# thu-nics/Rad-NeRF

Hardware: AMD Instinct MI355X
Metric: million samples/s fwd+bwd, 8192 rays, model_zoo_size=2; rgb L∞ vs ref (higher is better)
Workload: dtype f16/f32

## Files before the change

rad-nerf_amd/csrc/field_fwd_merged.hip:

```cpp
#include "rn_field.h"
#include "rn_merge.h"
#pragma clang fp contract(off)

static uint64_t g_level_pairing = 0;

namespace {

#define FM_KMAX 8
#define FM_LDS_K 4
static_assert(FM_KMAX == MB_KMAX, "k_field_fwd_merged reads the plan's descriptors");

template <int CACHE, bool ENC_M, bool GW>
__global__ void __launch_bounds__(1024)
k_field_fwd_merged(FieldArgs a, MergeArgs m) {
    extern __shared__ __attribute__((aligned(16))) rn_half sWm[];
    __shared__ LvTab sT;
    __shared__ int32_t sCh[2][2 + 2 * FM_KMAX];
    const int K = m.n_models, B = m.n_rays;
    if (!GW) {
        for (int k = 0; k < K; ++k)
            rn_block_copy16(sWm + (size_t)k * FIELD_FWD_FRAGS * RN_FRAG_HALFS,
                            a.frags + (size_t)k * FIELD_FRAGS * RN_FRAG_HALFS,
                            FIELD_FWD_FRAGS * RN_FRAG_BYTES);
    }
    lv_stage(sT, a.gm);
    const int waves = blockDim.x / RN_WAVE;
    const int wid = __builtin_amdgcn_readfirstlane(threadIdx.x / RN_WAVE);
    const int lane = rn_lane(), c = lane & 31, h = lane >> 5;
    int ticket = 0, n_chunks = 0;
    if (threadIdx.x == 0) { n_chunks = m.queue[1]; ticket = atomicAdd(m.queue + 2, 1); }

    auto mlp_tile = [&](const int32_t* ch, int u) {
        const int k = u % K, t = u / K;
        const int n_k = ch[2 + FM_KMAX + k];
        if (t * 32 >= n_k) return;
        rn_lds_order();
        const int i = t * 32 + c;
        const bool valid = i < n_k;
        const int64_t s = ch[2 + k] + (valid ? i : 0);
        FwdState st;
        float ux, uy, uz;
        constexpr int TC = ENC_M ? CACHE_READ_NT : CACHE;
        const rn_half* W = GW ? a.frags + (size_t)k * FIELD_FRAGS * RN_FRAG_HALFS
                              : sWm + (size_t)k * FIELD_FWD_FRAGS * RN_FRAG_HALFS;
        tile_forward_s<1, TC>(a, sT, W, s, valid, TC != CACHE_NONE ? cache_slot(a, s) : nullptr,
                              st, ux, uy, uz);
        if (valid && h == 0) {
            a.sigma[s] = expf(st.g0);
            a.rgb[3 * s + 0] = sigmoidf(st.out[0]);
            a.rgb[3 * s + 1] = sigmoidf(st.out[1]);
            a.rgb[3 * s + 2] = sigmoidf(st.out[2]);
        }
    };
    auto mlp_tiles = [&](const int32_t* ch) {
        int max_t = 0;
        for (int k = 0; k < K; ++k) max_t = max(max_t, (ch[2 + FM_KMAX + k] + 31) >> 5);
        return max_t * K;
    };

    bool prev_live = false;
    for (int it = 0;; ++it) {
        int32_t* cur = sCh[it & 1];
        const int32_t* prev = sCh[(it & 1) ^ 1];
        __syncthreads();
        if (threadIdx.x == 0) {
            const int ch = ticket;
            ticket = atomicAdd(m.queue + 2, 1);
            int4 d[CH_DESC / 4];
            if (ch < n_chunks) {
#pragma unroll
                for (int q = 0; q < CH_DESC / 4; ++q)
                    d[q] = reinterpret_cast<const int4*>(m.desc + (size_t)ch * CH_DESC)[q];
            }
            const int32_t* di = reinterpret_cast<const int32_t*>(d);
            cur[0] = ch < n_chunks ? di[CH_R0] : B;
            cur[1] = ch < n_chunks ? di[CH_R1] : B;
            for (int k = 0; k < K; ++k) {
                cur[2 + k] = di[ch_first(k)];
                cur[2 + FM_KMAX + k] = ch < n_chunks ? di[ch_count(k)] : 0;
            }
        }
        __syncthreads();
        const bool live = cur[0] < B;
        if (!ENC_M) {
            if (!live) break;
            const int nt = mlp_tiles(cur);
            for (int u = wid; u < nt; u += waves) mlp_tile(cur, u);
            continue;
        }
        if (!live && !prev_live) break;
        int p_base = 0, n_p = 0;
        if (live) { p_base = m.mstart[cur[0]]; n_p = m.mstart[cur[1]] - p_base; }
        const int nA = (n_p + 31) >> 5;
        const int nB = prev_live ? mlp_tiles(prev) : 0;
        for (int u = wid; u < nA + nB; u += waves) {
            if (u >= nA) { mlp_tile(prev, u - nA); continue; }
            const int q = u * 32 + c;
            const bool valid = q < n_p;
            const int64_t s = m.perm[p_base + (valid ? q : 0)];
            float x, y, z, dx, dy, dz;
            load_sample<1>(a, s, x, y, z, dx, dy, dz);
            const float ux = unit_coord(x, a.xyz_min[0], a.extent[0]);
            const float uy = unit_coord(y, a.xyz_min[1], a.extent[1]);
            const float uz = unit_coord(z, a.xyz_min[2], a.extent[2]);
            half8 e0, e1;
            encode_lane(a, sT, rn_rsrc(a.grid, a.grid_bytes), h, ux, uy, uz, valid, e0, e1);
            if (valid) { half8* fc = cache_slot(a, s); fc[0] = e0; fc[1] = e1; }
        }
        prev_live = live;
    }
}


__global__ void __launch_bounds__(256)
k_enc_prep(FieldArgs a, MergeArgs m, float4* __restrict__ prep) {
    const int P = m.mstart[m.n_rays];
    for (int p = blockIdx.x * blockDim.x + threadIdx.x; p < P; p += gridDim.x * blockDim.x) {
        const int s = m.perm[p];
        float x, y, z, dx, dy, dz;
        load_sample<1>(a, s, x, y, z, dx, dy, dz);
        prep[p] = make_float4(unit_coord(x, a.xyz_min[0], a.extent[0]),
                              unit_coord(y, a.xyz_min[1], a.extent[1]),
                              unit_coord(z, a.xyz_min[2], a.extent[2]), __int_as_float(s));
    }
}

__global__ void __launch_bounds__(256)
k_field_encode_levels(FieldArgs a, MergeArgs m, const float4* __restrict__ prep,
                      int32_t* __restrict__ xq, uint64_t pairing) {
    __shared__ LvTab sT;
    lv_stage(sT, a.gm);
    __syncthreads();
    const int g = blockIdx.x & 7;
    if (xq && threadIdx.x == 0) {
        uint32_t xcc;
        asm volatile("s_getreg_b32 %0, hwreg(HW_REG_XCC_ID, 0, 4)" : "=s"(xcc));
        atomicAdd(xq + 8 * g + (int)(xcc & 7u), 1);
        atomicMin(reinterpret_cast<unsigned long long*>(xq + 64) + g,
                  (unsigned long long)__builtin_amdgcn_s_memrealtime());
    }
    const int la = (int)((pairing >> (8 * g)) & 15u), lb = (int)((pairing >> (8 * g + 4)) & 15u);
    const int P = m.mstart[m.n_rays];
    const int nt = (P + 31) >> 5;
    const int nb = (int)(gridDim.x >> 3), j = (int)(blockIdx.x >> 3);
    const int t0 = (int)((int64_t)nt * j / nb), t1 = (int)((int64_t)nt * (j + 1) / nb);
    const int wid = __builtin_amdgcn_readfirstlane(threadIdx.x >> 6), waves = blockDim.x >> 6;
    const int lane = rn_lane(), c = lane & 31, h = lane >> 5;
    const __amdgpu_buffer_rsrc_t rs = rn_rsrc(a.grid, a.grid_bytes);
    const LvConst LA = lv_const_uniform(sT, a.gm, la), LB = lv_const_uniform(sT, a.gm, lb);
#pragma unroll 1
    for (int ph = 0; ph < 2; ++ph) {
        const LvConst& LC = ph ? LB : LA;
        uint32_t* const out = const_cast<uint32_t*>(a.planes) + (size_t)(ph ? lb : la) * a.plane_stride;
        for (int t = t0 + 2 * wid; t < t1; t += 2 * waves) {
            const bool v0 = t * 32 + c < P;
            const bool v1 = t + 1 < t1 && (t + 1) * 32 + c < P;
            const bool valid = h ? v1 : v0;
            const int p = (t + h) * 32 + c;
            const float4 q = prep[valid ? p : 0];
            const uint32_t v = encode_tiles(a, rs, h, LC, q.x, q.y, q.z, v0, v1);
            if (valid) __builtin_nontemporal_store(v, out + __float_as_int(q.w));
        }
    }
    if (xq) {
        __syncthreads();
        if (threadIdx.x == 0)
            atomicMax(reinterpret_cast<unsigned long long*>(xq + 80) + g,
                      (unsigned long long)__builtin_amdgcn_s_memrealtime());
    }
}

__global__ void __launch_bounds__(1024)
k_field_mlp_planes(FieldArgs a, int K) {
    extern __shared__ __attribute__((aligned(16))) rn_half sWm[];
    __shared__ LvTab sT;
    __shared__ int32_t sSeg[2][FM_KMAX];
    lv_stage(sT, a.gm);
    if (threadIdx.x < K) {
        sSeg[0][threadIdx.x] = a.seg_base[threadIdx.x];
        sSeg[1][threadIdx.x] = a.seg_count[threadIdx.x];
    }
    int first[FM_KMAX + 1];
    first[0] = 0;
    for (int k = 0; k < K; ++k)
        first[k + 1] = first[k] + ((__builtin_amdgcn_readfirstlane(a.seg_count[k]) + 31) >> 5);
    const int T = first[K];
    const int u0 = (int)((int64_t)T * blockIdx.x / gridDim.x);
    const int u1 = (int)((int64_t)T * (blockIdx.x + 1) / gridDim.x);
    if (u0 >= u1) return;
    int k_lo = 0, k_hi = 0;
    for (int k = 0; k < K; ++k) {
        if (first[k + 1] <= u0) k_lo = k + 1;
        if (first[k] < u1) k_hi = k;
    }
    const int wid = __builtin_amdgcn_readfirstlane(threadIdx.x >> 6), waves = blockDim.x >> 6;
    const int lane = rn_lane(), c = lane & 31, h = lane >> 5;
    for (int kb = k_lo; kb <= k_hi; kb += FM_LDS_K) {
        const int ke = min(k_hi, kb + FM_LDS_K - 1);
        __syncthreads();
        for (int k = kb; k <= ke; ++k)
            rn_block_copy16(sWm + (size_t)(k - kb) * FIELD_FWD_FRAGS * RN_FRAG_HALFS,
                            a.frags + (size_t)k * FIELD_FRAGS * RN_FRAG_HALFS,
                            FIELD_FWD_FRAGS * RN_FRAG_BYTES);
        __syncthreads();
        const int ua = max(u0, first[kb]), ub = min(u1, first[ke + 1]);
        for (int u = ua + wid; u < ub; u += waves) {
            int k = kb;
            while (k < ke && u >= first[k + 1]) ++k;
            const int t = u - first[k];
            const int n_k = sSeg[1][k];
            const int i = t * 32 + c;
            const bool valid = i < n_k;
            const int64_t s = sSeg[0][k] + (valid ? i : 0);
            FwdState st;
            float ux, uy, uz;
            rn_lds_order();
            tile_forward_s<1, CACHE_PLANES>(a, sT, sWm + (size_t)(k - kb) * FIELD_FWD_FRAGS * RN_FRAG_HALFS,
                                            s, valid, a.feat ? cache_slot(a, s) : nullptr, st,
                                            ux, uy, uz);
            if (valid && h == 0) {
                a.sigma[s] = expf(st.g0);
                a.rgb[3 * s + 0] = sigmoidf(st.out[0]);
                a.rgb[3 * s + 1] = sigmoidf(st.out[1]);
                a.rgb[3 * s + 2] = sigmoidf(st.out[2]);
            }
        }
    }
}

}

extern "C" {

int rn_set_level_pairing(uint64_t pairing) {
    if (pairing != 0) {
        uint32_t seen = 0;
        for (int i = 0; i < 16; ++i) seen |= 1u << ((pairing >> (4 * i)) & 15u);
        RN_CHECK_ARG(seen == 0xffffu, "pairing: every level exactly once");
    }
    g_level_pairing = pairing;
    return 0;
}

int rn_field_fwd_merged(const float* ts, const int32_t* ray_of, const float* rays_o,
                        const float* rays_d, const int32_t* seg_base, const int32_t* seg_count,
                        const int32_t* chunk_desc, int32_t* queue,
                        int64_t n_rays, int32_t n_models, const void* grid_f16,
                        const uint32_t* level_offset, const uint32_t* level_hsize,
                        const uint32_t* level_res, const float* level_scale,
                        const float* xyz_min, const float* extent, const void* frags,
                        float* sigma, float* rgb, void* feat_cache, const int32_t* mstart,
                        const int32_t* perm, int32_t blocks, int32_t threads, void* stream) {
    RN_CHECK_ARG(n_rays >= 1 && n_models >= 1 && n_models <= FM_KMAX && blocks >= 1,
                 "bad sizes (n_models <= 8)");
    RN_CHECK_ARG(threads >= 64 && threads <= 1024 && threads % 64 == 0, "threads: 64..1024, waves");
    RN_CHECK_ARG(ts && ray_of && rays_o && rays_d && seg_base && seg_count &&
                 chunk_desc && queue && grid_f16 && level_offset && level_hsize && level_res &&
                 level_scale && xyz_min && extent && frags && sigma && rgb, "null pointer");
    RN_CHECK_ARG(!(mstart || perm) || (mstart && perm && feat_cache),
                 "merged-order encoding needs mstart, perm and the encoding cache");
    FieldArgs a{};
    field_args_grid(a, grid_f16, level_offset, level_hsize, level_res, level_scale, xyz_min, extent,
                    frags);
    field_args_compact(a, ts, ray_of, rays_o, rays_d, seg_base, seg_count);
    a.sigma = sigma; a.rgb = rgb; a.feat = (rn_half*)feat_cache;
    MergeArgs m{};
    m.desc = chunk_desc; m.queue = queue;
    m.mstart = mstart; m.perm = perm;
    m.n_rays = (int)n_rays; m.n_models = n_models;
    const bool gw = n_models > FM_LDS_K;
    const size_t lds = gw ? 0 : (size_t)n_models * FIELD_FWD_FRAGS * RN_FRAG_BYTES;
    hipStream_t st = (hipStream_t)stream;
    RN_CHECK_HIP(hipMemsetAsync(queue + 2, 0, sizeof(int32_t), st), "ticket reset");
#define RN_FM_LAUNCH(C, E)                                                                     \
    do {                                                                                       \
        if (gw) k_field_fwd_merged<C, E, true><<<blocks, threads, 0, st>>>(a, m);              \
        else k_field_fwd_merged<C, E, false><<<blocks, threads, lds, st>>>(a, m);              \
    } while (0)
    if (mstart) RN_FM_LAUNCH(CACHE_WRITE, true);
    else if (feat_cache) RN_FM_LAUNCH(CACHE_WRITE, false);
    else RN_FM_LAUNCH(CACHE_NONE, false);
#undef RN_FM_LAUNCH
    RN_CHECK_LAUNCH();
    return 0;
}

int rn_field_fwd_levels(const float* ts, const int32_t* ray_of, const float* rays_o,
                        const float* rays_d, const int32_t* seg_base, const int32_t* seg_count,
                        int64_t n_rays, int32_t n_models, const void* grid_f16,
                        const uint32_t* level_offset, const uint32_t* level_hsize,
                        const uint32_t* level_res, const float* level_scale,
                        const float* xyz_min, const float* extent, const void* frags,
                        float* sigma, float* rgb, void* feat_cache, const int32_t* mstart,
                        const int32_t* perm, uint32_t* planes, int64_t plane_stride, void* prep,
                        int32_t prep_ready, int32_t enc_blocks, int32_t mlp_blocks, int32_t* xq,
                        void* stream) {
    RN_CHECK_ARG(n_rays >= 1 && n_models >= 1 && n_models <= FM_KMAX && plane_stride >= 1,
                 "bad sizes (n_models <= 8)");
    RN_CHECK_ARG(enc_blocks >= 8 && enc_blocks % 8 == 0 && mlp_blocks >= 1,
                 "bad launch (enc_blocks: a multiple of 8)");
    RN_CHECK_ARG(ts && ray_of && rays_o && rays_d && seg_base && seg_count && grid_f16 &&
                 level_offset && level_hsize && level_res && level_scale && xyz_min && extent &&
                 frags && sigma && rgb && mstart && perm && planes && prep, "null pointer");
    FieldArgs a{};
    field_args_grid(a, grid_f16, level_offset, level_hsize, level_res, level_scale, xyz_min, extent,
                    frags);
    field_args_compact(a, ts, ray_of, rays_o, rays_d, seg_base, seg_count);
    a.sigma = sigma; a.rgb = rgb; a.feat = (rn_half*)feat_cache;
    a.planes = planes; a.plane_stride = plane_stride;
    MergeArgs m{};
    m.mstart = mstart; m.perm = perm; m.n_rays = (int)n_rays; m.n_models = n_models;
    hipStream_t st = (hipStream_t)stream;
    if (xq) {
        RN_CHECK_HIP(hipMemsetAsync(xq, 0, 64 * sizeof(int32_t), st), "probe reset");
        RN_CHECK_HIP(hipMemsetAsync(xq + 64, 0xff, 16 * sizeof(int32_t), st), "probe reset");
        RN_CHECK_HIP(hipMemsetAsync(xq + 80, 0, 16 * sizeof(int32_t), st), "probe reset");
    }
    if (!prep_ready) k_enc_prep<<<1024, 256, 0, st>>>(a, m, (float4*)prep);
    uint64_t pairing = g_level_pairing;
    if (pairing == 0)
        for (int g = 0; g < 8; ++g) pairing |= (uint64_t)(g | ((RN_L - 1 - g) << 4)) << (8 * g);
    k_field_encode_levels<<<enc_blocks, 256, 0, st>>>(a, m, (const float4*)prep, xq, pairing);
    k_field_mlp_planes<<<mlp_blocks, 1024,
                         (size_t)min(n_models, FM_LDS_K) * FIELD_FWD_FRAGS * RN_FRAG_BYTES, st>>>(
        a, n_models);
    RN_CHECK_LAUNCH();
    return 0;
}

}
```

rad-nerf_amd/csrc/rn_field.h:

```cpp
#pragma once
#include "rn_mlp.h"
#pragma clang fp contract(off)

#define RN_L 16
#define FIELD_FWD_FRAGS 24
#define FIELD_FRAGS 46
#define FIELD_PARAMS 9472
#define FIELD_DW_TILES 12
#ifndef FWD_MIN_WAVES
#define FWD_MIN_WAVES 2
#endif

struct GridMeta {
    uint32_t offset[RN_L];
    uint32_t hsize[RN_L];
    uint32_t res[RN_L];
    float scale[RN_L];
    uint32_t dense_mask;
    uint32_t pow2_mask;
};

struct FieldArgs {
    const float* xyzs; const float* dirs;
    const float* ts; const int32_t* ray_of; const float* rays_o; const float* rays_d;
    const int32_t* seg_base; const int32_t* seg_count;
    int64_t n_fixed;
    const rn_half* grid;
    float* grid_grad;
    const rn_half* frags;
    float* dw;
    float* sigma; float* rgb;
    const float* dsigma; const float* drgb;
    rn_half* feat;
    const uint32_t* planes;
    int64_t plane_stride;
    float xyz_min[3]; float extent[3];
    uint32_t grid_bytes;
    int dbg;
    GridMeta gm;
};

namespace {


__device__ __forceinline__ void sample_range(const FieldArgs& a, int MODE, int k, int64_t& base,
                                             int64_t& n) {
    if (MODE == 0) { base = 0; n = a.n_fixed; }
    else { base = a.seg_base[k]; n = a.seg_count[k]; }
}

template <int MODE>
__device__ __forceinline__ void load_sample(const FieldArgs& a, int64_t s, float& x, float& y,
                                            float& z, float& dx, float& dy, float& dz) {
    if (MODE == 0) {
        x = a.xyzs[3 * s]; y = a.xyzs[3 * s + 1]; z = a.xyzs[3 * s + 2];
        dx = a.dirs[3 * s]; dy = a.dirs[3 * s + 1]; dz = a.dirs[3 * s + 2];
    } else {
        const int r = (rn_dbg(a.dbg) & 8192) ? 0 : a.ray_of[s];
        const float t = a.ts[s];
        dx = a.rays_d[3 * r]; dy = a.rays_d[3 * r + 1]; dz = a.rays_d[3 * r + 2];
        x = fmaf(t, dx, a.rays_o[3 * r]);
        y = fmaf(t, dy, a.rays_o[3 * r + 1]);
        z = fmaf(t, dz, a.rays_o[3 * r + 2]);
    }
}

__device__ __forceinline__ float unit_coord(float v, float mn, float ext) {
    return fminf(fmaxf((v - mn) / ext, 0.0f), 1.0f);
}

__device__ __forceinline__ int lane_level(int q, int h) { return 2 * h + (q & 1) + 4 * (q >> 1); }

struct LvTab {
    uint32_t off[RN_L];
    uint32_t hs[RN_L];
    uint32_t res[RN_L];
    uint32_t res2[RN_L];
    float sc[RN_L];
};

__device__ __forceinline__ void lv_stage(LvTab& t, const GridMeta& gm) {
    const int i = threadIdx.x;
    if (i < RN_L) {
        t.off[i] = gm.offset[i]; t.hs[i] = gm.hsize[i]; t.res[i] = gm.res[i]; t.sc[i] = gm.scale[i];
        t.res2[i] = gm.res[i] * gm.res[i];
    }
}

struct LvConst {
    uint32_t off, hs, res, res2;
    float sc;
    bool dense;
};

__device__ __forceinline__ LvConst lv_const(const LvTab& T, const GridMeta& gm, int l) {
    LvConst c;
    c.off = T.off[l]; c.hs = T.hs[l]; c.res = T.res[l]; c.res2 = T.res2[l]; c.sc = T.sc[l];
    c.dense = (gm.dense_mask >> l) & 1u;
    return c;
}

__device__ __forceinline__ uint32_t grid_index(const LvConst& c, uint32_t x, uint32_t y, uint32_t z) {
    const uint32_t di = x + __umul24(y, c.res) + __umul24(z, c.res2);
    const uint32_t hi = x ^ (y * 2654435761u) ^ (z * 805459861u);
    const uint32_t dm = di >= c.hs ? di - c.hs : di;
    return c.dense ? dm : (hi & (c.hs - 1u));
}

struct LevelPos { uint32_t gx, gy, gz; float fx, fy, fz; };

__device__ __forceinline__ LevelPos level_pos(float sc, float ux, float uy, float uz) {
    LevelPos p;
    float px = fmaf(sc, ux, 0.5f), py = fmaf(sc, uy, 0.5f), pz = fmaf(sc, uz, 0.5f);
    auto cvt_flr = [](float v) {
        int r;
        asm("v_cvt_flr_i32_f32 %0, %1" : "=v"(r) : "v"(v));
        return (uint32_t)r;
    };
    p.gx = cvt_flr(px); p.gy = cvt_flr(py); p.gz = cvt_flr(pz);
    p.fx = __builtin_amdgcn_fractf(px); p.fy = __builtin_amdgcn_fractf(py); p.fz = __builtin_amdgcn_fractf(pz);
    return p;
}

__device__ __forceinline__ float corner_weight(const LevelPos& p, int c) {
    float w = 1.0f;
    w *= (c & 1) ? p.fx : 1.0f - p.fx;
    w *= (c & 2) ? p.fy : 1.0f - p.fy;
    w *= (c & 4) ? p.fz : 1.0f - p.fz;
    return w;
}

__device__ __forceinline__ uint32_t corner_index(const LvConst& c, const LevelPos& p, int corner) {
    return grid_index(c, p.gx + (corner & 1), p.gy + ((corner >> 1) & 1), p.gz + ((corner >> 2) & 1));
}

__device__ __forceinline__ __amdgpu_buffer_rsrc_t rn_rsrc(const void* p, uint32_t bytes) {
    return __builtin_amdgcn_make_buffer_rsrc(const_cast<void*>(p), (short)0, (int)bytes,
                                             0x00020000);
}

#define RN_OOB 0x80000000u

__device__ __forceinline__ void encode_lane(const FieldArgs& a, const LvTab& T,
                                            __amdgpu_buffer_rsrc_t rs, int h, float ux, float uy,
                                            float uz, bool valid, half8& e0, half8& e1) {
    float f[16];
    const bool load = valid && !(rn_dbg(a.dbg) & 128);
#pragma unroll
    for (int lb = 0; lb < RN_L; lb += 4) {
        uint32_t GX[4], ROW[4][4];
        float FX[4], FY[4], FZ[4];
#pragma unroll
        for (int up = 0; up < 4; up += 2) {
            const LvConst lm = lv_const(T, a.gm, lb + up + h);
            const LevelPos p = level_pos(lm.sc, ux, uy, uz);
            uint32_t rw[4];
            if (lm.dense) {
                const uint32_t b = __umul24(p.gy, lm.res) + __umul24(p.gz, lm.res2);
#pragma unroll
                for (int r = 0; r < 4; ++r)
                    rw[r] = b + ((r & 1) ? lm.res : 0u) + ((r >> 1) ? lm.res2 : 0u);
            } else {
                const uint32_t y0 = p.gy * 2654435761u, z0 = p.gz * 805459861u;
                const uint32_t y1 = y0 + 2654435761u, z1 = z0 + 805459861u;
#pragma unroll
                for (int r = 0; r < 4; ++r) rw[r] = ((r & 1) ? y1 : y0) ^ ((r >> 1) ? z1 : z0);
            }
            auto xch = [&](uint32_t v, uint32_t& lo, uint32_t& hi) {
                const auto r2 = __builtin_amdgcn_permlane32_swap(v, v, false, false);
                lo = r2[0]; hi = r2[1];
            };
            uint32_t t0, t1;
            xch(p.gx, GX[up], GX[up + 1]);
            xch(__float_as_uint(p.fx), t0, t1); FX[up] = __uint_as_float(t0); FX[up + 1] = __uint_as_float(t1);
            xch(__float_as_uint(p.fy), t0, t1); FY[up] = __uint_as_float(t0); FY[up + 1] = __uint_as_float(t1);
            xch(__float_as_uint(p.fz), t0, t1); FZ[up] = __uint_as_float(t0); FZ[up + 1] = __uint_as_float(t1);
#pragma unroll
            for (int r = 0; r < 4; ++r) xch(rw[r], ROW[up][r], ROW[up + 1][r]);
        }
        uint32_t off[16];
#pragma unroll
        for (int u = 0; u < 4; ++u) {
            const LvConst lc = lv_const(T, a.gm, lb + u);
            const uint32_t x = GX[u] + (uint32_t)h;
            uint32_t idx[4];
            if (lc.dense) {
#pragma unroll
                for (int r = 0; r < 4; ++r) {
                    const uint32_t d = x + ROW[u][r];
                    idx[r] = min(d, d - lc.hs);
                }
            } else {
#pragma unroll
                for (int r = 0; r < 4; ++r) idx[r] = (x ^ ROW[u][r]) & (lc.hs - 1u);
            }
            const uint32_t ob = load ? lc.off : (RN_OOB >> 2);
#pragma unroll
            for (int r = 0; r < 4; ++r) off[4 * u + r] = (ob + idx[r]) << 2;
        }
        uint32_t raw[16];
#pragma unroll
        for (int i = 0; i < 16; ++i) raw[i] = __builtin_amdgcn_raw_buffer_load_b32(rs, off[i], 0, 0);
#pragma unroll
        for (int u = 0; u < 4; ++u) {
            float a0 = 0.f, a1 = 0.f;
            const float wx = h ? FX[u] : 1.0f - FX[u];
            const float wy0 = 1.0f - FY[u], wz0 = 1.0f - FZ[u];
            const float wxy0 = wx * wy0, wxy1 = wx * FY[u];
#pragma unroll
            for (int r = 0; r < 4; ++r) {
                const float w = ((r & 1) ? wxy1 : wxy0) * ((r >> 1) ? FZ[u] : wz0);
                const uint32_t v = raw[4 * u + r];
                a0 = fmaf(w, (float)__builtin_bit_cast(rn_half, (uint16_t)(v & 0xffffu)), a0);
                a1 = fmaf(w, (float)__builtin_bit_cast(rn_half, (uint16_t)(v >> 16)), a1);
            }
            const auto s0 = __builtin_amdgcn_permlane32_swap(__float_as_uint(a0), __float_as_uint(a0), false, false);
            const auto s1 = __builtin_amdgcn_permlane32_swap(__float_as_uint(a1), __float_as_uint(a1), false, false);
            const float v0 = __uint_as_float(s0[0]) + __uint_as_float(s0[1]);
            const float v1 = __uint_as_float(s1[0]) + __uint_as_float(s1[1]);
            const int L = lb + u, q = (L & 1) + 2 * (L >> 2);
            if (((L >> 1) & 1) == h) { f[2 * q] = v0; f[2 * q + 1] = v1; }
        }
#ifndef FWD_NO_SCHED_BARRIER
        __builtin_amdgcn_sched_barrier(0);
#endif
    }
#pragma unroll
    for (int j = 0; j < 8; ++j) { e0[j] = (rn_half)f[j]; e1[j] = (rn_half)f[8 + j]; }
}

__device__ __forceinline__ LvConst lv_const_uniform(const LvTab& T, const GridMeta& gm, int l) {
    const LvConst c = lv_const(T, gm, l);
    LvConst u;
    u.off = (uint32_t)__builtin_amdgcn_readfirstlane((int)c.off);
    u.hs = (uint32_t)__builtin_amdgcn_readfirstlane((int)c.hs);
    u.res = (uint32_t)__builtin_amdgcn_readfirstlane((int)c.res);
    u.res2 = (uint32_t)__builtin_amdgcn_readfirstlane((int)c.res2);
    u.sc = __int_as_float(__builtin_amdgcn_readfirstlane(__float_as_int(c.sc)));
    u.dense = c.dense;
    return u;
}

__device__ __forceinline__ uint32_t encode_tiles(const FieldArgs& a, __amdgpu_buffer_rsrc_t rs,
                                                 int h, const LvConst& L, float ux, float uy,
                                                 float uz, bool valid0, bool valid1) {
    uint32_t GX[2], ROW[2][4];
    float FX[2], FY[2], FZ[2];
    const int dn = __builtin_amdgcn_readfirstlane((int)L.dense);
    {
        const LevelPos p = level_pos(L.sc, ux, uy, uz);
        uint32_t rw[4];
        if (dn) {
            const uint32_t b = __umul24(p.gy, L.res) + __umul24(p.gz, L.res2);
#pragma unroll
            for (int r = 0; r < 4; ++r) rw[r] = b + ((r & 1) ? L.res : 0u) + ((r >> 1) ? L.res2 : 0u);
        } else {
            const uint32_t y0 = p.gy * 2654435761u, z0 = p.gz * 805459861u;
            const uint32_t y1 = y0 + 2654435761u, z1 = z0 + 805459861u;
#pragma unroll
            for (int r = 0; r < 4; ++r) rw[r] = ((r & 1) ? y1 : y0) ^ ((r >> 1) ? z1 : z0);
        }
        auto xch = [&](uint32_t v, uint32_t& lo, uint32_t& hi) {
            const auto r2 = __builtin_amdgcn_permlane32_swap(v, v, false, false);
            lo = r2[0]; hi = r2[1];
        };
        uint32_t t0, t1;
        xch(p.gx, GX[0], GX[1]);
        xch(__float_as_uint(p.fx), t0, t1); FX[0] = __uint_as_float(t0); FX[1] = __uint_as_float(t1);
        xch(__float_as_uint(p.fy), t0, t1); FY[0] = __uint_as_float(t0); FY[1] = __uint_as_float(t1);
        xch(__float_as_uint(p.fz), t0, t1); FZ[0] = __uint_as_float(t0); FZ[1] = __uint_as_float(t1);
#pragma unroll
        for (int r = 0; r < 4; ++r) xch(rw[r], ROW[0][r], ROW[1][r]);
    }
    const bool noload = rn_dbg(a.dbg) & 128;
    uint32_t off[8];
#pragma unroll
    for (int u = 0; u < 2; ++u) {
        const uint32_t x = GX[u] + (uint32_t)h;
        const uint32_t ob = ((u ? valid1 : valid0) && !noload) ? L.off : (RN_OOB >> 2);
        if (dn) {
#pragma unroll
            for (int r = 0; r < 4; ++r) {
                const uint32_t d = x + ROW[u][r];
                off[4 * u + r] = (ob + min(d, d - L.hs)) << 2;
            }
        } else {
#pragma unroll
            for (int r = 0; r < 4; ++r) off[4 * u + r] = (ob + ((x ^ ROW[u][r]) & (L.hs - 1u))) << 2;
        }
    }
    uint32_t raw[8];
#pragma unroll
    for (int i = 0; i < 8; ++i) raw[i] = __builtin_amdgcn_raw_buffer_load_b32(rs, off[i], 0, 0);
    uint32_t res = 0u;
#pragma unroll
    for (int u = 0; u < 2; ++u) {
        float a0 = 0.f, a1 = 0.f;
        const float wx = h ? FX[u] : 1.0f - FX[u];
        const float wy0 = 1.0f - FY[u], wz0 = 1.0f - FZ[u];
        const float wxy0 = wx * wy0, wxy1 = wx * FY[u];
#pragma unroll
        for (int r = 0; r < 4; ++r) {
            const float w = ((r & 1) ? wxy1 : wxy0) * ((r >> 1) ? FZ[u] : wz0);
            const uint32_t v = raw[4 * u + r];
            a0 = fmaf(w, (float)__builtin_bit_cast(rn_half, (uint16_t)(v & 0xffffu)), a0);
            a1 = fmaf(w, (float)__builtin_bit_cast(rn_half, (uint16_t)(v >> 16)), a1);
        }
        const auto s0 = __builtin_amdgcn_permlane32_swap(__float_as_uint(a0), __float_as_uint(a0), false, false);
        const auto s1 = __builtin_amdgcn_permlane32_swap(__float_as_uint(a1), __float_as_uint(a1), false, false);
        const float v0 = __uint_as_float(s0[0]) + __uint_as_float(s0[1]);
        const float v1 = __uint_as_float(s1[0]) + __uint_as_float(s1[1]);
        const uint32_t pk = (uint32_t)__builtin_bit_cast(uint16_t, (rn_half)v0) |
                            ((uint32_t)__builtin_bit_cast(uint16_t, (rn_half)v1) << 16);
        if (u == h) res = pk;
    }
    return res;
}

__device__ __forceinline__ half8 sh_lane(float dx, float dy, float dz, int h) {
    const float n = sqrtf(dx * dx + dy * dy + dz * dz);
    const float x = fmaf((dx / n + 1.0f) / 2.0f, 2.0f, -1.0f);
    const float y = fmaf((dy / n + 1.0f) / 2.0f, 2.0f, -1.0f);
    const float z = fmaf((dz / n + 1.0f) / 2.0f, 2.0f, -1.0f);
    const float xy = x * y, xz = x * z, yz = y * z, x2 = x * x, y2 = y * y, z2 = z * z;
    float o[16];
    o[0] = 0.28209479177387814f;
    o[1] = -0.48860251190291987f * y;
    o[2] = 0.48860251190291987f * z;
    o[3] = -0.48860251190291987f * x;
    o[4] = 1.0925484305920792f * xy;
    o[5] = -1.0925484305920792f * yz;
    o[6] = 0.94617469575755997f * z2 - 0.31539156525251999f;
    o[7] = -1.0925484305920792f * xz;
    o[8] = 0.54627421529603959f * x2 - 0.54627421529603959f * y2;
    o[9] = 0.59004358992664352f * y * (-3.0f * x2 + y2);
    o[10] = 2.8906114426405538f * xy * z;
    o[11] = 0.45704579946446572f * y * (1.0f - 5.0f * z2);
    o[12] = 0.3731763325901154f * z * (5.0f * z2 - 3.0f);
    o[13] = 0.45704579946446572f * x * (1.0f - 5.0f * z2);
    o[14] = 1.4453057213202769f * z * (x2 - y2);
    o[15] = 0.59004358992664352f * x * (-x2 + 3.0f * y2);
    half8 r;
#pragma unroll
    for (int j = 0; j < 8; ++j) {
        const int c0 = 8 * (j >> 2) + (j & 3);
        r[j] = (rn_half)(h ? o[c0 + 4] : o[c0]);
    }
    return r;
}

struct FwdState {
    half8 e0, e1;
    half8 h1[4];
    half8 gin;
    half8 sh;
    half8 r1[4], r2[4];
    float g0;
    f32x16 out;
};

__device__ __forceinline__ void mlp_forward(const rn_half* W, FwdState& st) {
    f32x16 a0 = rn_zero16(), a1 = rn_zero16();
    a0 = rn_mfma(rn_frag(W, 0), st.e0, a0); a0 = rn_mfma(rn_frag(W, 1), st.e1, a0);
    a1 = rn_mfma(rn_frag(W, 2), st.e0, a1); a1 = rn_mfma(rn_frag(W, 3), st.e1, a1);
    rn_acc_to_frags<true>(a0, st.h1[0], st.h1[1]);
    rn_acc_to_frags<true>(a1, st.h1[2], st.h1[3]);
    f32x16 g = rn_zero16();
#pragma unroll
    for (int q = 0; q < 4; ++q) g = rn_mfma(rn_frag(W, 4 + q), st.h1[q], g);
    half8 gk1;
    rn_acc_to_frags<false>(g, st.gin, gk1);
    st.g0 = g[8];
    a0 = rn_zero16(); a1 = rn_zero16();
    a0 = rn_mfma(rn_frag(W, 8), st.sh, a0); a0 = rn_mfma(rn_frag(W, 9), st.gin, a0);
    a1 = rn_mfma(rn_frag(W, 10), st.sh, a1); a1 = rn_mfma(rn_frag(W, 11), st.gin, a1);
    rn_acc_to_frags<true>(a0, st.r1[0], st.r1[1]);
    rn_acc_to_frags<true>(a1, st.r1[2], st.r1[3]);
    a0 = rn_zero16(); a1 = rn_zero16();
#pragma unroll
    for (int q = 0; q < 4; ++q) {
        a0 = rn_mfma(rn_frag(W, 12 + q), st.r1[q], a0);
        a1 = rn_mfma(rn_frag(W, 16 + q), st.r1[q], a1);
    }
    rn_acc_to_frags<true>(a0, st.r2[0], st.r2[1]);
    rn_acc_to_frags<true>(a1, st.r2[2], st.r2[3]);
    st.out = rn_zero16();
#pragma unroll
    for (int q = 0; q < 4; ++q) st.out = rn_mfma(rn_frag(W, 20 + q), st.r2[q], st.out);
}

__device__ __forceinline__ float sigmoidf(float x) { return 1.0f / (1.0f + expf(-x)); }

enum { CACHE_NONE = 0, CACHE_WRITE = 1, CACHE_READ = 2,
       CACHE_READ_NT = 3,
       CACHE_PLANES = 4 };

template <int CACHE>
__device__ __forceinline__ void tile_forward_pos(const FieldArgs& a, const LvTab& T, const rn_half* W,
                                                 float x, float y, float z, float dx, float dy,
                                                 float dz, bool valid, half8* fc, FwdState& st,
                                                 float& ux, float& uy, float& uz);

template <int MODE, int CACHE>
__device__ __forceinline__ void tile_forward_s(const FieldArgs& a, const LvTab& T, const rn_half* W,
                                               int64_t s, bool valid, half8* fc, FwdState& st,
                                               float& ux, float& uy, float& uz) {
    float x = 0.f, y = 0.f, z = 0.f, dx = 1.f, dy = 0.f, dz = 0.f;
    if (CACHE == CACHE_PLANES) {
        const int h = rn_lane() >> 5;
        typedef uint32_t u4v __attribute__((ext_vector_type(4)));
        u4v w0 = {0u, 0u, 0u, 0u}, w1 = {0u, 0u, 0u, 0u};
        if (valid) {
            const uint32_t* pl = a.planes + s;
#pragma unroll
            for (int q = 0; q < 4; ++q) {
                w0[q] = pl[(size_t)lane_level(q, h) * a.plane_stride];
                w1[q] = pl[(size_t)lane_level(q + 4, h) * a.plane_stride];
            }
        }
        st.e0 = __builtin_bit_cast(half8, w0); st.e1 = __builtin_bit_cast(half8, w1);
    }
    if (valid) load_sample<MODE>(a, s, x, y, z, dx, dy, dz);
    tile_forward_pos<CACHE>(a, T, W, x, y, z, dx, dy, dz, valid, fc, st, ux, uy, uz);
}

template <int CACHE>
__device__ __forceinline__ void tile_forward_rays(const FieldArgs& a, const LvTab& T,
                                                  const rn_half* W, int64_t s, bool valid,
                                                  half8* fc, const float* sRays, int r0, int nr,
                                                  FwdState& st, float& ux, float& uy, float& uz) {
    float x = 0.f, y = 0.f, z = 0.f, dx = 1.f, dy = 0.f, dz = 0.f;
    if (valid) {
        const int r = a.ray_of[s];
        const float t = a.ts[s];
        const uint32_t q = (uint32_t)(r - r0);
        float ox, oy, oz;
        if (q < (uint32_t)nr) {
            typedef __attribute__((address_space(3))) const float lds_f;
            lds_f* p = (lds_f*)sRays + 6 * q;
            ox = p[0]; oy = p[1]; oz = p[2]; dx = p[3]; dy = p[4]; dz = p[5];
        } else {
            ox = a.rays_o[3 * r]; oy = a.rays_o[3 * r + 1]; oz = a.rays_o[3 * r + 2];
            dx = a.rays_d[3 * r]; dy = a.rays_d[3 * r + 1]; dz = a.rays_d[3 * r + 2];
        }
        x = fmaf(t, dx, ox);
        y = fmaf(t, dy, oy);
        z = fmaf(t, dz, oz);
    }
    tile_forward_pos<CACHE>(a, T, W, x, y, z, dx, dy, dz, valid, fc, st, ux, uy, uz);
}

template <int CACHE>
__device__ __forceinline__ void tile_forward_pos(const FieldArgs& a, const LvTab& T, const rn_half* W,
                                                 float x, float y, float z, float dx, float dy,
                                                 float dz, bool valid, half8* fc, FwdState& st,
                                                 float& ux, float& uy, float& uz) {
    const int h = rn_lane() >> 5;
    ux = unit_coord(x, a.xyz_min[0], a.extent[0]);
    uy = unit_coord(y, a.xyz_min[1], a.extent[1]);
    uz = unit_coord(z, a.xyz_min[2], a.extent[2]);
    if (CACHE == CACHE_PLANES) {
        if (valid && fc) { fc[0] = st.e0; fc[1] = st.e1; }
    } else if (CACHE == CACHE_READ || CACHE == CACHE_READ_NT) {
        st.e0 = rn_zero8(); st.e1 = rn_zero8();
        if (valid && CACHE == CACHE_READ) { st.e0 = fc[0]; st.e1 = fc[1]; }
        if (valid && CACHE == CACHE_READ_NT) {
            st.e0 = __builtin_nontemporal_load(fc);
            st.e1 = __builtin_nontemporal_load(fc + 1);
        }
    } else {
        if (rn_dbg(a.dbg) & 256) { st.e0 = rn_zero8(); st.e1 = rn_zero8(); asm volatile("" :: "v"(ux), "v"(uy), "v"(uz)); }
        else encode_lane(a, T, rn_rsrc(a.grid, a.grid_bytes), h, ux, uy, uz, valid, st.e0, st.e1);
        if (CACHE == CACHE_WRITE && valid) { fc[0] = st.e0; fc[1] = st.e1; }
    }
    st.sh = sh_lane(dx, dy, dz, h);
    if (rn_dbg(a.dbg) & 4096) {
        st.out = rn_zero16(); st.g0 = 0.f;
        asm volatile("" :: "v"(st.e0), "v"(st.e1), "v"(st.sh));
    } else {
        mlp_forward(W, st);
    }
}

__device__ __forceinline__ half8* cache_slot(const FieldArgs& a, int64_t s) {
    return reinterpret_cast<half8*>(a.feat) + ((s >> 5) * 64 + (s & 31) + 32 * (rn_lane() >> 5)) * 2;
}

template <int MODE, int CACHE>
__device__ __forceinline__ void tile_forward(const FieldArgs& a, const LvTab& T, const rn_half* W,
                                             int64_t base, int64_t n, int64_t tile, FwdState& st,
                                             bool& valid, int64_t& s, float& ux, float& uy,
                                             float& uz) {
    const int lane = rn_lane(), c = lane & 31;
    const int64_t i = tile * 32 + c;
    valid = i < n;
    s = base + (valid ? i : 0);
    half8* fc = CACHE == CACHE_NONE ? nullptr
              : reinterpret_cast<half8*>(a.feat) + (((base >> 5) + tile) * 64 + lane) * 2;
    tile_forward_s<MODE, CACHE>(a, T, W, s, valid, fc, st, ux, uy, uz);
}

int fill_args(FieldArgs& a, const float* xyz_min, const float* extent, const uint32_t* offsets,
              const uint32_t* hsize, const uint32_t* res, const float* scale) {
    for (int d = 0; d < 3; ++d) { a.xyz_min[d] = xyz_min[d]; a.extent[d] = extent[d]; }
    a.gm.dense_mask = 0;
    a.gm.pow2_mask = 0;
    a.grid_bytes = 4u * (offsets[RN_L - 1] + hsize[RN_L - 1]);
    for (int l = 0; l < RN_L; ++l) {
        a.gm.offset[l] = offsets[l]; a.gm.hsize[l] = hsize[l]; a.gm.res[l] = res[l];
        a.gm.scale[l] = scale[l];
        const uint64_t r = res[l];
        if (r * r * r <= (uint64_t)hsize[l]) a.gm.dense_mask |= 1u << l;
        if (hsize[l] && (hsize[l] & (hsize[l] - 1u)) == 0) a.gm.pow2_mask |= 1u << l;
    }
    return 0;
}

static void field_args_grid(FieldArgs& a, const void* grid_f16, const uint32_t* level_offset,
                            const uint32_t* level_hsize, const uint32_t* level_res,
                            const float* level_scale, const float* xyz_min, const float* extent,
                            const void* frags) {
    fill_args(a, xyz_min, extent, level_offset, level_hsize, level_res, level_scale);
    a.dbg = rn_debug_flags_internal();
    a.grid = (const rn_half*)grid_f16; a.frags = (const rn_half*)frags;
}

static void field_args_compact(FieldArgs& a, const float* ts, const int32_t* ray_of,
                               const float* rays_o, const float* rays_d, const int32_t* seg_base,
                               const int32_t* seg_count) {
    a.ts = ts; a.ray_of = ray_of; a.rays_o = rays_o; a.rays_d = rays_d;
    a.seg_base = seg_base; a.seg_count = seg_count;
}

}
```

Before: 1211.

## Software-pipeline plane loads and ray lookups in the planes MLP kernel

Rewrites the per-tile loop of the planes MLP kernel into a software pipeline. The plane feature words for the next tile and the ray index two tiles ahead are loaded while the current tile runs its MLP, and output stores are deferred by one iteration. This is meant to hide global-memory latency, and it also drops the unused LDS grid-table staging and the position and unit-coordinate computation the planes path did not need. The cost is more registers held across iterations, which may reduce occupancy, plus a new 32-bit offset limit on plane_stride.

```diff
diff --git a/rad-nerf_amd/csrc/field_fwd_merged.hip b/rad-nerf_amd/csrc/field_fwd_merged.hip
--- a/rad-nerf_amd/csrc/field_fwd_merged.hip
+++ b/rad-nerf_amd/csrc/field_fwd_merged.hip
@@ -173,9 +173,7 @@
 __global__ void __launch_bounds__(1024)
 k_field_mlp_planes(FieldArgs a, int K) {
     extern __shared__ __attribute__((aligned(16))) rn_half sWm[];
-    __shared__ LvTab sT;
     __shared__ int32_t sSeg[2][FM_KMAX];
-    lv_stage(sT, a.gm);
     if (threadIdx.x < K) {
         sSeg[0][threadIdx.x] = a.seg_base[threadIdx.x];
         sSeg[1][threadIdx.x] = a.seg_count[threadIdx.x];
@@ -204,27 +202,61 @@
                             FIELD_FWD_FRAGS * RN_FRAG_BYTES);
         __syncthreads();
         const int ua = max(u0, first[kb]), ub = min(u1, first[ke + 1]);
-        for (int u = ua + wid; u < ub; u += waves) {
-            int k = kb;
+        auto locate = [&](int u, int& k, int& s) {
+            k = kb;
             while (k < ke && u >= first[k + 1]) ++k;
-            const int t = u - first[k];
-            const int n_k = sSeg[1][k];
-            const int i = t * 32 + c;
-            const bool valid = i < n_k;
-            const int64_t s = sSeg[0][k] + (valid ? i : 0);
+            const int i = (u - first[k]) * 32 + c;
+            const bool valid = i < sSeg[1][k];
+            s = sSeg[0][k] + (valid ? i : 0);
+            return valid;
+        };
+        struct Ahead { int k, s, r; bool valid, live; };
+        auto look = [&](int un, Ahead& t) {
+            t.live = un < ub;
+            if (t.live) t.valid = locate(un, t.k, t.s);
+        };
+        int u = ua + wid;
+        if (u >= ub) continue;
+        PlaneTile cur;
+        Ahead use = {0, 0, 0, false, false}, far = use;
+        look(u, use);
+        planes_issue(a, use.k, use.s, use.valid, planes_issue_ray(a, use.s), cur);
+        look(u + waves, use);
+        if (use.live) {
+            use.r = planes_issue_ray(a, use.s);
+            asm volatile("" :: "v"(use.r));
+        }
+        asm volatile("" :: "v"(cur.w1));
+        float o_sigma = 0.f, o_r = 0.f, o_g = 0.f, o_b = 0.f;
+        int64_t o_s = 0;
+        bool o_valid = false;
+        auto store_out = [&]() {
+            if (o_valid && h == 0) {
+                a.sigma[o_s] = o_sigma;
+                a.rgb[3 * o_s + 0] = o_r;
+                a.rgb[3 * o_s + 1] = o_g;
+                a.rgb[3 * o_s + 2] = o_b;
+            }
+        };
+        for (; u < ub; u += waves) {
+            PlaneTile nxt;
+            look(u + 2 * waves, far);
+            if (use.live) planes_issue(a, use.k, use.s, use.valid, use.r, nxt);
+            if (far.live) far.r = planes_issue_ray(a, far.s);
+            store_out();
+            __builtin_amdgcn_sched_barrier(0);
             FwdState st;
-            float ux, uy, uz;
             rn_lds_order();
-            tile_forward_s<1, CACHE_PLANES>(a, sT, sWm + (size_t)(k - kb) * FIELD_FWD_FRAGS * RN_FRAG_HALFS,
-                                            s, valid, a.feat ? cache_slot(a, s) : nullptr, st,
-                                            ux, uy, uz);
-            if (valid && h == 0) {
-                a.sigma[s] = expf(st.g0);
-                a.rgb[3 * s + 0] = sigmoidf(st.out[0]);
-                a.rgb[3 * s + 1] = sigmoidf(st.out[1]);
-                a.rgb[3 * s + 2] = sigmoidf(st.out[2]);
-            }
-        }
+            tile_forward_planes(a, sWm + (size_t)(cur.k - kb) * FIELD_FWD_FRAGS * RN_FRAG_HALFS, cur,
+                                st);
+            o_valid = cur.valid; o_s = cur.s;
+            o_sigma = expf(st.g0);
+            o_r = sigmoidf(st.out[0]); o_g = sigmoidf(st.out[1]); o_b = sigmoidf(st.out[2]);
+            __builtin_amdgcn_sched_barrier(0);
+            if (use.live) cur = nxt;
+            use = far;
+        }
+        store_out();
     }
 }
 
@@ -297,6 +329,7 @@
                         void* stream) {
     RN_CHECK_ARG(n_rays >= 1 && n_models >= 1 && n_models <= FM_KMAX && plane_stride >= 1,
                  "bad sizes (n_models <= 8)");
+    RN_CHECK_ARG(plane_stride <= (int64_t)1 << 28, "plane_stride: at most 2^28 sample slots");
     RN_CHECK_ARG(enc_blocks >= 8 && enc_blocks % 8 == 0 && mlp_blocks >= 1,
                  "bad launch (enc_blocks: a multiple of 8)");
     RN_CHECK_ARG(ts && ray_of && rays_o && rays_d && seg_base && seg_count && grid_f16 &&
diff --git a/rad-nerf_amd/csrc/rn_field.h b/rad-nerf_amd/csrc/rn_field.h
--- a/rad-nerf_amd/csrc/rn_field.h
+++ b/rad-nerf_amd/csrc/rn_field.h
@@ -392,8 +392,7 @@
 __device__ __forceinline__ float sigmoidf(float x) { return 1.0f / (1.0f + expf(-x)); }
 
 enum { CACHE_NONE = 0, CACHE_WRITE = 1, CACHE_READ = 2,
-       CACHE_READ_NT = 3,
-       CACHE_PLANES = 4 };
+       CACHE_READ_NT = 3 };
 
 template <int CACHE>
 __device__ __forceinline__ void tile_forward_pos(const FieldArgs& a, const LvTab& T, const rn_half* W,
@@ -406,20 +405,6 @@
                                                int64_t s, bool valid, half8* fc, FwdState& st,
                                                float& ux, float& uy, float& uz) {
     float x = 0.f, y = 0.f, z = 0.f, dx = 1.f, dy = 0.f, dz = 0.f;
-    if (CACHE == CACHE_PLANES) {
-        const int h = rn_lane() >> 5;
-        typedef uint32_t u4v __attribute__((ext_vector_type(4)));
-        u4v w0 = {0u, 0u, 0u, 0u}, w1 = {0u, 0u, 0u, 0u};
-        if (valid) {
-            const uint32_t* pl = a.planes + s;
-#pragma unroll
-            for (int q = 0; q < 4; ++q) {
-                w0[q] = pl[(size_t)lane_level(q, h) * a.plane_stride];
-                w1[q] = pl[(size_t)lane_level(q + 4, h) * a.plane_stride];
-            }
-        }
-        st.e0 = __builtin_bit_cast(half8, w0); st.e1 = __builtin_bit_cast(half8, w1);
-    }
     if (valid) load_sample<MODE>(a, s, x, y, z, dx, dy, dz);
     tile_forward_pos<CACHE>(a, T, W, x, y, z, dx, dy, dz, valid, fc, st, ux, uy, uz);
 }
@@ -459,9 +444,7 @@
     ux = unit_coord(x, a.xyz_min[0], a.extent[0]);
     uy = unit_coord(y, a.xyz_min[1], a.extent[1]);
     uz = unit_coord(z, a.xyz_min[2], a.extent[2]);
-    if (CACHE == CACHE_PLANES) {
-        if (valid && fc) { fc[0] = st.e0; fc[1] = st.e1; }
-    } else if (CACHE == CACHE_READ || CACHE == CACHE_READ_NT) {
+    if (CACHE == CACHE_READ || CACHE == CACHE_READ_NT) {
         st.e0 = rn_zero8(); st.e1 = rn_zero8();
         if (valid && CACHE == CACHE_READ) { st.e0 = fc[0]; st.e1 = fc[1]; }
         if (valid && CACHE == CACHE_READ_NT) {
@@ -484,6 +467,49 @@
 
 __device__ __forceinline__ half8* cache_slot(const FieldArgs& a, int64_t s) {
     return reinterpret_cast<half8*>(a.feat) + ((s >> 5) * 64 + (s & 31) + 32 * (rn_lane() >> 5)) * 2;
+}
+
+typedef uint32_t rn_u4v __attribute__((ext_vector_type(4)));
+typedef float rn_f3v __attribute__((ext_vector_type(3)));
+
+struct PlaneTile {
+    int k;
+    int s;
+    bool valid;
+    rn_u4v w0, w1;
+    rn_f3v d;
+};
+
+__device__ __forceinline__ int planes_issue_ray(const FieldArgs& a, int s) {
+    return (rn_dbg(a.dbg) & 8192) ? 0 : a.ray_of[s];
+}
+
+__device__ __forceinline__ void planes_issue(const FieldArgs& a, int k, int s, bool valid, int r,
+                                             PlaneTile& p) {
+    const int h = rn_lane() >> 5;
+    p.k = k; p.s = s; p.valid = valid;
+    p.d = rn_f3v{a.rays_d[3 * r], a.rays_d[3 * r + 1], a.rays_d[3 * r + 2]};
+    const uint32_t off = ((uint32_t)s + (uint32_t)(2 * h) * (uint32_t)a.plane_stride) * 4u;
+#pragma unroll
+    for (int q = 0; q < 8; ++q) {
+        const char* base = reinterpret_cast<const char*>(a.planes + (size_t)lane_level(q, 0) * a.plane_stride);
+        const uint32_t w = *reinterpret_cast<const uint32_t*>(base + off);
+        if (q < 4) p.w0[q] = w; else p.w1[q - 4] = w;
+    }
+}
+
+__device__ __forceinline__ void tile_forward_planes(const FieldArgs& a, const rn_half* W,
+                                                    const PlaneTile& p, FwdState& st) {
+    const int h = rn_lane() >> 5;
+    st.e0 = __builtin_bit_cast(half8, p.w0); st.e1 = __builtin_bit_cast(half8, p.w1);
+    if (p.valid && a.feat) { half8* fc = cache_slot(a, p.s); fc[0] = st.e0; fc[1] = st.e1; }
+    st.sh = sh_lane(p.d[0], p.d[1], p.d[2], h);
+    if (rn_dbg(a.dbg) & 4096) {
+        st.out = rn_zero16(); st.g0 = 0.f;
+        asm volatile("" :: "v"(st.e0), "v"(st.e1), "v"(st.sh));
+    } else {
+        mlp_forward(W, st);
+    }
 }
 
 template <int MODE, int CACHE>
```

New measurement: 1217 (median of 6 runs). No clear change (+0.4%).
